# ChuyueL/advanced-hpc-lbm

Measured on NVIDIA B200. Metric: MLUPS (d2q9-bgk lattice updates per second / 1e6), higher is better.
Workload: dtype f32

## Files before the change

### advanced-hpc-lbm_b200/csrc/lbm_gpu.cu

```cuda
#include "lbm_gpu.h"
#include "lbm_kernels.cuh"
#include "lbm_cluster.cuh"
#include "lbm_tb2.cuh"
#include "lbm_tb3.cuh"
#include "lbm_pairs.cuh"
#include "lbm_f16.cuh"

#include <unistd.h>

#include <algorithm>
#include <cmath>
#include <cstdarg>
#include <cstdio>
#include <cstdlib>
#include <cstring>
#include <exception>
#include <memory>
#include <mutex>
#include <string>
#include <vector>

namespace {

thread_local std::string g_error;
// ... 1700 lines not shown
    s.rows = (int)nrows;
    const long long ar = (long long)params->ny - 2;
    s.accel_row = (ar >= row0 && ar < row0 + nrows) ? (int)(ar - row0) : LBM_NO_ROW;
    g->select_kernel();
    g->alloc_slab(s);
    if (g->kernel == LBM_GPU_KERNEL_TMA) g->make_tensor_maps(s);
    g->load_slab(s, cells_aos_rows, obstacles_rows, 0);
    if (nrows == params->ny) { g->connect_local(); g->prepare(); }
  } catch (const CudaError& e) {
    return fail("lbm_gpu_create_slab: %s", e.what.c_str());
  } catch (const std::exception& e) {
    return fail("lbm_gpu_create_slab: %s", e.what());
  }
  *out = reinterpret_cast<lbm_gpu*>(static_cast<GridBase*>(g.release()));
  return 0;
}

int lbm_gpu_ipc_export(lbm_gpu* h, void* desc) {
  if (!desc) return fail("lbm_gpu_ipc_export: NULL descriptor");
  return guarded<float>(h, "lbm_gpu_ipc_export", [&](Grid<float>& g) {
    if (g.slabs.size() != 1) throw CudaError{"only a one-slab handle can be exported"};
    if (g.f16) throw CudaError{"a LBM_GPU_STORE_F16 lattice cannot be shared between processes"};
    Slab<float>& s = g.slabs[0];
    CK(cudaSetDevice(s.device));
    IpcDesc d;
    memset(&d, 0, sizeof d);
    d.magic = kIpcMagic;
    d.elem_size = 4;
    d.device = s.device;
    d.pid = (int32_t)getpid();
    d.nx = g.prm.nx; d.pitch = g.pitch; d.rows = s.rows;
    d.row0 = s.row0;
    d.win_addr = (unsigned long long)(uintptr_t)s.win;
    d.win_bytes = s.win_bytes;
    d.off_sync = s.off_sync;
    d.off_gmask = s.off_gmask;
    d.steps_done = (unsigned long long)g.steps_done;
    d.passes_done = (unsigned long long)g.passes_done;
    d.local_free_cells = s.free_cells;
    d.cur = g.cur;
    d.tb2_ok = g.k7_fits(s.rows) ? 1 : 0;
    CK(cudaIpcGetMemHandle(&d.handle, s.win));
    cudaDeviceProp prop;
    CK(cudaGetDeviceProperties(&prop, s.device));
    memcpy(d.gpu_uuid, prop.uuid.bytes, 16);
    memset(desc, 0, LBM_GPU_IPC_DESC_BYTES);
    memcpy(desc, &d, sizeof d);
  });
}

namespace {
void ipc_connect_impl(Grid<float>& g, const IpcDesc& dn, const IpcDesc& up, bool ring_k7) {
  if (g.slabs.size() != 1) throw CudaError{"only a one-slab handle can be connected"};
  if (g.f16) throw CudaError{"a LBM_GPU_STORE_F16 lattice cannot be shared between processes"};
  Slab<float>& s = g.slabs[0];
  CK(cudaSetDevice(s.device));
  const long long ny = g.prm.ny;
  for (const IpcDesc* d : {&dn, &up}) {
    if (d->magic != kIpcMagic || d->elem_size != 4) throw CudaError{"bad neighbour descriptor"};
    if (d->nx != g.prm.nx || d->pitch != g.pitch) throw CudaError{"neighbour descriptor is for another grid width"};
    if (d->steps_done != (unsigned long long)g.steps_done || d->passes_done != (unsigned long long)g.passes_done ||
        d->cur != g.cur)
      throw CudaError{"neighbour is at a different timestep"};
  }
  cudaDeviceProp my_prop;
  CK(cudaGetDeviceProperties(&my_prop, s.device));
  for (const IpcDesc* d : {&dn, &up})
    if (memcmp(d->gpu_uuid, my_prop.uuid.bytes, 16) == 0 &&
        !(d->pid == (int32_t)getpid() && d->win_addr == (unsigned long long)(uintptr_t)s.win))
      throw CudaError{"a neighbouring slab runs on the same physical GPU: kernels that wait on one another "
                      "must not share a device (use lbm_gpu_create with n_gpus slabs in one process instead)"};
  if ((dn.row0 + dn.rows) % ny != s.row0 % ny) throw CudaError{"descriptor 'below' does not hold row0-1"};
  if ((s.row0 + s.rows) % ny != up.row0 % ny) throw CudaError{"descriptor 'above' does not hold row0+nrows"};
  auto map = [&](const IpcDesc& d, int slot) -> char* {
    if (d.pid == (int32_t)getpid()) {
      char* p = (char*)(uintptr_t)d.win_addr;
      if (p == s.win) return p;
      if (d.device == s.device)
        throw CudaError{"two slabs ordered by device-side flags must not share a GPU"};
      int can = 0;
      CK(cudaDeviceCanAccessPeer(&can, s.device, d.device));
      if (!can) throw CudaError{"peer access between the selected GPUs is not available"};
      cudaError_t e = cudaDeviceEnablePeerAccess(d.device, 0);
      if (e != cudaSuccess && e != cudaErrorPeerAccessAlreadyEnabled) CK(e);
      cudaGetLastError();
      return p;
    }
    if (g.use_pool()) {
      std::lock_guard<std::mutex> lock(g_window_mutex);
      for (auto& c : g_ipc_cache)
        if (c.device == s.device && memcmp(&c.handle, &d.handle, sizeof d.handle) == 0) return (char*)c.ptr;
    }
    void* p = nullptr;
    CK(cudaIpcOpenMemHandle(&p, d.handle, cudaIpcMemLazyEnablePeerAccess));
    if (g.use_pool()) {
      std::lock_guard<std::mutex> lock(g_window_mutex);
      g_ipc_cache.push_back({d.handle, s.device, p});
    } else {
      s.ipc_mapped[slot] = p;
    }
    return (char*)p;
  };
  for (const IpcDesc* d : {&dn, &up})
    if (d->win_bytes != s.win_bytes || d->off_sync != s.off_sync || d->off_gmask != s.off_gmask)
      throw CudaError{"neighbour window layout differs"};
  s.dn_win = map(dn, 0);
  s.up_win = (memcmp(&dn.handle, &up.handle, sizeof dn.handle) == 0 && dn.pid == up.pid) ? s.dn_win : map(up, 1);
  unsigned long long* dn_sync = (unsigned long long*)(s.dn_win + dn.off_sync);
  unsigned long long* up_sync = (unsigned long long*)(s.up_win + up.off_sync);
  s.dn_flag = dn_sync + kFlagFromAbove;
  s.up_flag = up_sync + kFlagFromBelow;
  s.dn_abort = dn_sync + kAbort;
  s.up_abort = up_sync + kAbort;
  s.dn_gmask = (uint32_t*)(s.dn_win + dn.off_gmask) + g.mask_pitch;
  s.up_gmask = (uint32_t*)(s.up_win + up.off_gmask);
  g.multi = true;
  g.use_flags = true;
  g.select_kernel(true, ring_k7);
  g.connected = true;
}
}

int lbm_gpu_ipc_connect(lbm_gpu* h, const void* desc_below, const void* desc_above) {
  if (!desc_below || !desc_above) return fail("lbm_gpu_ipc_connect: NULL descriptor");
  return guarded<float>(h, "lbm_gpu_ipc_connect", [&](Grid<float>& g) {
    IpcDesc dn, up;
    memcpy(&dn, desc_below, sizeof dn);
    memcpy(&up, desc_above, sizeof up);
    ipc_connect_impl(g, dn, up, false);
  });
}

int lbm_gpu_ipc_connect_all(lbm_gpu* h, const void* descs, int n) {
  if (!descs || n < 1) return fail("lbm_gpu_ipc_connect_all: bad argument");
  return guarded<float>(h, "lbm_gpu_ipc_connect_all", [&](Grid<float>& g) {
    if (g.slabs.size() != 1) throw CudaError{"only a one-slab handle can be connected"};
    Slab<float>& s = g.slabs[0];
    std::vector<IpcDesc> all(n);
    for (int i = 0; i < n; i++) memcpy(&all[i], (const char*)descs + (size_t)i * LBM_GPU_IPC_DESC_BYTES, sizeof(IpcDesc));
    const long long ny = g.prm.ny;
    long long rows_total = 0, free_total = 0;
    int below = -1, above = -1;
    bool all_k7 = true;
    for (int i = 0; i < n; i++) {
      const IpcDesc& d = all[i];
      if (d.magic != kIpcMagic) throw CudaError{"bad descriptor in the list"};
      rows_total += d.rows;
      free_total += d.local_free_cells;
      all_k7 = all_k7 && d.tb2_ok;
      if ((d.row0 + d.rows) % ny == s.row0 % ny) below = i;
      if ((s.row0 + s.rows) % ny == d.row0 % ny) above = i;
    }
    if (rows_total != ny) throw CudaError{"the descriptors do not cover the grid's rows exactly once"};
    if (below < 0 || above < 0) throw CudaError{"no descriptor holds the rows next to this slab"};
    ipc_connect_impl(g, all[below], all[above], all_k7);
    g.global_free_cells = free_total;
  });
}

int lbm_gpu_ipc_prepare(lbm_gpu* h) {
  return guarded<float>(h, "lbm_gpu_ipc_prepare", [&](Grid<float>& g) { g.prepare(); });
}

int lbm_gpu_run(lbm_gpu* h, int n_steps, float* av_vels_out) {
  return run_impl<float>(h, n_steps, av_vels_out, nullptr, "lbm_gpu_run");
}
int lbm_gpu_run_f64(lbm_gpu* h, int n_steps, double* av_vels_out) {
  return run_impl<double>(h, n_steps, av_vels_out, nullptr, "lbm_gpu_run_f64");
}
int lbm_gpu_run_batch(lbm_gpu* const* handles, int n, int n_steps, float* av_vels_out) {
  return run_batch_impl(handles, n, n_steps, av_vels_out);
}
int lbm_gpu_run_sums(lbm_gpu* h, int n_steps, double* sums_out) {
  if (!h) return fail("lbm_gpu_run_sums: NULL handle");
  if (reinterpret_cast<GridBase*>(h)->is_f64()) return run_impl<double>(h, n_steps, nullptr, sums_out, "lbm_gpu_run_sums");
  return run_impl<float>(h, n_steps, nullptr, sums_out, "lbm_gpu_run_sums");
}

int lbm_gpu_set_global_free_cells(lbm_gpu* h, long long free_cells) {
  if (!h) return fail("lbm_gpu_set_global_free_cells: NULL handle");
  if (free_cells < 1) return fail("lbm_gpu_set_global_free_cells: count must be positive");
  GridBase* b = reinterpret_cast<GridBase*>(h);
  if (b->is_f64()) static_cast<Grid<double>*>(b)->global_free_cells = free_cells;
  else static_cast<Grid<float>*>(b)->global_free_cells = free_cells;
  return 0;
}

int lbm_gpu_download(lbm_gpu* h, float* out) {
  if (!out) return fail("lbm_gpu_download: NULL output");
  return guarded<float>(h, "lbm_gpu_download", [&](Grid<float>& g) {
    long long rows = 0;
    for (auto& s : g.slabs) rows += s.rows;
    g.download_rows(g.slabs[0].row0, rows, out);
  });
}
int lbm_gpu_download_f64(lbm_gpu* h, double* out) {
  if (!out) return fail("lbm_gpu_download_f64: NULL output");
  return guarded<double>(h, "lbm_gpu_download_f64", [&](Grid<double>& g) {
    long long rows = 0;
    for (auto& s : g.slabs) rows += s.rows;
    g.download_rows(g.slabs[0].row0, rows, out);
  });
}
int lbm_gpu_download_rows(lbm_gpu* h, long long row0, long long nrows, float* out) {
  if (!out || nrows < 0) return fail("lbm_gpu_download_rows: bad argument");
  return guarded<float>(h, "lbm_gpu_download_rows", [&](Grid<float>& g) { g.download_rows(row0, nrows, out); });
}

int lbm_gpu_final_fields(lbm_gpu* h, long long row0, long long nrows, float* ux, float* uy, float* u, float* p) {
  if (nrows < 0) return fail("lbm_gpu_final_fields: bad argument");
  return guarded<float>(h, "lbm_gpu_final_fields", [&](Grid<float>& g) { g.final_fields(row0, nrows, ux, uy, u, p); });
}
int lbm_gpu_final_fields_f64(lbm_gpu* h, long long row0, long long nrows, double* ux, double* uy, double* u, double* p) {
  if (nrows < 0) return fail("lbm_gpu_final_fields_f64: bad argument");
  return guarded<double>(h, "lbm_gpu_final_fields_f64", [&](Grid<double>& g) { g.final_fields(row0, nrows, ux, uy, u, p); });
}

int lbm_gpu_av_velocity(lbm_gpu* h, float* av_out) {
  if (!av_out) return fail("lbm_gpu_av_velocity: NULL output");
  return guarded<float>(h, "lbm_gpu_av_velocity", [&](Grid<float>& g) {
    *av_out = (float)(g.av_velocity_sum() / (double)g.divisor());
  });
}
int lbm_gpu_av_velocity_f64(lbm_gpu* h, double* av_out) {
  if (!av_out) return fail("lbm_gpu_av_velocity_f64: NULL output");
  return guarded<double>(h, "lbm_gpu_av_velocity_f64", [&](Grid<double>& g) {
    *av_out = g.av_velocity_sum() / (double)g.divisor();
  });
}

int lbm_gpu_digest(lbm_gpu* h, double* total_density, unsigned long long* checksum) {
  if (!h) return fail("lbm_gpu_digest: NULL handle");
  if (reinterpret_cast<GridBase*>(h)->is_f64())
    return guarded<double>(h, "lbm_gpu_digest", [&](Grid<double>& g) { g.digest(total_density, checksum); });
  return guarded<float>(h, "lbm_gpu_digest", [&](Grid<float>& g) { g.digest(total_density, checksum); });
}

int lbm_gpu_upload(lbm_gpu* h, const float* cells_aos) {
  if (!cells_aos) return fail("lbm_gpu_upload: NULL input");
  return guarded<float>(h, "lbm_gpu_upload", [&](Grid<float>& g) {
    const int cur = g.cur;
    const long long base = g.slabs[0].row0;
    for (auto& s : g.slabs) g.upload_cells(s, cells_aos + (size_t)(s.row0 - base) * g.prm.nx * 9, cur);
    if (!g.slab_mode || g.slabs[0].rows == g.prm.ny) g.prepare();
  });
}
int lbm_gpu_upload_f64(lbm_gpu* h, const double* cells_aos) {
  if (!cells_aos) return fail("lbm_gpu_upload_f64: NULL input");
  return guarded<double>(h, "lbm_gpu_upload_f64", [&](Grid<double>& g) {
    const int cur = g.cur;
    for (auto& s : g.slabs) g.upload_cells(s, cells_aos + (size_t)s.row0 * g.prm.nx * 9, cur);
    g.prepare();
  });
}

int lbm_gpu_get_info(lbm_gpu* h, lbm_gpu_info* info) {
  if (!h || !info) return fail("lbm_gpu_get_info: NULL argument");
  memset(info, 0, sizeof *info);
  GridBase* b = reinterpret_cast<GridBase*>(h);
  auto fill = [&](auto& g) {
    info->nx = g.prm.nx; info->ny = g.prm.ny;
    info->n_gpus = (int)g.slabs.size();
    info->is_f64 = g.is_f64();
    info->kernel = g.kernel;
    info->pitch = g.pitch;
    info->local_free_cells = g.local_free_cells();
    info->free_cells = g.divisor();
    info->local_row0 = g.slabs[0].row0;
    long long rows = 0;
    size_t bytes = 0;
    for (auto& s : g.slabs) { rows += s.rows; bytes = std::max(bytes, s.bytes + kStagingBytes); }
    info->local_rows = rows;
    info->steps_done = g.steps_done;
    info->kernel_launches = g.launches;
    info->last_run_device_ms = g.last_run_ms;
    info->last_step_kernel_ms = g.last_step_ms;
    info->device_bytes = bytes;
  };
  if (b->is_f64()) fill(*static_cast<Grid<double>*>(b));
  else fill(*static_cast<Grid<float>*>(b));
  return 0;
}

int lbm_gpu_host_alloc(size_t bytes, void** out) {
  if (!out) return fail("lbm_gpu_host_alloc: NULL argument");
  *out = nullptr;
  cudaError_t e = cudaHostAlloc(out, bytes, cudaHostAllocPortable);
  if (e != cudaSuccess) {
    cudaGetLastError();
    return fail("lbm_gpu_host_alloc: %s", cudaGetErrorString(e));
  }
  return 0;
}

void lbm_gpu_host_free(void* p) {
  if (p) cudaFreeHost(p);
}

void lbm_gpu_destroy(lbm_gpu* h) {
  if (!h) return;
  delete reinterpret_cast<GridBase*>(h);
}

}
```

### advanced-hpc-lbm_b200/csrc/lbm_tb2.cuh

```cuda
#pragma once
#include "lbm_kernels.cuh"

namespace lbm {

#ifndef LBM_TB2_THREADS
#define LBM_TB2_THREADS 96
#endif
#define LBM_TB2_SPAN (LBM_TB2_THREADS * 4)
#define LBM_TB2_PAD 4
#define LBM_TB2_ROWF (LBM_TB2_SPAN + 2 * LBM_TB2_PAD)
#define LBM_TB2_MAX_WOUT (LBM_TB2_SPAN - 8)
#ifndef LBM_TB2_MIN_BLOCKS
#define LBM_TB2_MIN_BLOCKS 4
#endif

struct Tb2Smem {
  float in[2][9][LBM_TB2_ROWF];
  float r013[2][3][LBM_TB2_ROWF];
  float r256[3][3][LBM_TB2_ROWF];
  float r78[2][LBM_TB2_ROWF];
  unsigned long long mbar[2];
  unsigned long long mbar_free;
};
static_assert(sizeof(Tb2Smem) * LBM_TB2_MIN_BLOCKS <= 225 * 1024, "LBM_TB2_MIN_BLOCKS blocks of shared memory per SM");
static_assert((LBM_TB2_ROWF * sizeof(float)) % 16 == 0, "staged rows must keep 16-byte alignment");

struct Tb2Args {
  StepArgs<float> s;
  const uint32_t* ghost_mask;
  unsigned long long* av2;
  int wout;
  int span;
  int seg_rows;
  int n_big;
  int big_rows;
  int seg_rows_tail;
  unsigned long long* av3;
};

__device__ __forceinline__ void tb2_mbar_wait(unsigned long long* bar, const uint32_t parity) {
  const uint32_t addr = smem_u32(bar);
  uint32_t done = 0;
  while (!done)
    asm volatile("{ .reg .pred p; mbarrier.try_wait.parity.shared::cta.b64 p, [%1], %2; selp.b32 %0, 1, 0, p; }"
                 : "=r"(done) : "r"(addr), "r"(parity) : "memory");
}

__device__ __forceinline__ void tb2_bulk_load(float* dst_smem, const float* src, const uint32_t bytes,
                                              unsigned long long* bar) {
  asm volatile("cp.async.bulk.shared::cluster.global.mbarrier::complete_tx::bytes [%0], [%1], %2, [%3];"
               ::"r"(smem_u32(dst_smem)), "l"(src), "r"(bytes), "r"(smem_u32(bar)) : "memory");
}

template <bool PERIODIC = false>
__device__ __forceinline__ const float* tb2_row_ptr(const StepArgs<float>& a, const int k, int row) {
  if (PERIODIC) {
    row = (row < 0) ? row + a.rows : (row >= a.rows) ? row - a.rows : row;
  } else {
    if (row < 0) return a.ghost_s + (long long)((-1 - row) * 9 + k) * a.pitch;
    if (row >= a.rows) return a.ghost_n + (long long)((row - a.rows) * 9 + k) * a.pitch;
  }
  if (row == a.accel_row && k != 0 && k != 2 && k != 4) {
    const int idx = (k == 1) ? 0 : (k == 3) ? 1 : k - 3;
    return a.side_src + (long long)idx * a.pitch;
  }
  return a.src + (long long)k * a.plane_stride + (long long)row * a.pitch;
}

template <typename Smem>
__device__ __forceinline__ void tb2_expect(Smem& sm, const int stage, const int span) {
  asm volatile("mbarrier.arrive.expect_tx.shared::cta.b64 _, [%0], %1;" ::"r"(smem_u32(&sm.mbar[stage])),
               "r"((uint32_t)(9 * span * sizeof(float))) : "memory");
}
__device__ __forceinline__ int tb2_plane_of_thread() {
  const int nwarps = (int)blockDim.x >> 5, w = (int)threadIdx.x >> 5, lane = (int)threadIdx.x & 31;
  const int k = w + nwarps * lane;
  return (k < 9) ? k : -1;
}
template <bool PERIODIC = false, typename Smem>
__device__ __forceinline__ void tb2_issue(const StepArgs<float>& a, Smem& sm, const int stage, const int r,
                                          const int s0, const int span, const int k) {
  if (k < 0) return;
  unsigned long long* bar = &sm.mbar[stage];
  const int dy = (k == 2 || k == 5 || k == 6) ? -1 : (k == 4 || k == 7 || k == 8) ? 1 : 0;
  const float* row = tb2_row_ptr<PERIODIC>(a, k, r + dy);
  float* dst = &sm.in[stage][k][LBM_TB2_PAD];
  int col = s0, left = span;
  while (left > 0) {
    const int n = min(left, a.nx - col);
    tb2_bulk_load(dst, row + col, (uint32_t)n * 4u, bar);
    dst += n;
    left -= n;
    col = 0;
  }
}

__device__ __forceinline__ void tb2_get(const float* row, const int c0, float& v0, float& v1, float& v2, float& v3) {
  const float4 v = *reinterpret_cast<const float4*>(row + LBM_TB2_PAD + c0);
  v0 = v.x; v1 = v.y; v2 = v.z; v3 = v.w;
}
__device__ __forceinline__ void tb2_get_west(const float* row, const int c0, float& v0, float& v1, float& v2, float& v3) {
  const float4 v = *reinterpret_cast<const float4*>(row + LBM_TB2_PAD + c0);
  v0 = row[LBM_TB2_PAD + c0 - 1]; v1 = v.x; v2 = v.y; v3 = v.z;
}
__device__ __forceinline__ void tb2_get_east(const float* row, const int c0, float& v0, float& v1, float& v2, float& v3) {
  const float4 v = *reinterpret_cast<const float4*>(row + LBM_TB2_PAD + c0);
  v0 = v.y; v1 = v.z; v2 = v.w; v3 = row[LBM_TB2_PAD + c0 + 4];
}
__device__ __forceinline__ void tb2_ring_read_done(Tb2Smem& sm) {
  __syncwarp();
  if ((threadIdx.x & 31) == 0)
    asm volatile("mbarrier.arrive.shared::cta.b64 _, [%0];" ::"r"(smem_u32(&sm.mbar_free)) : "memory");
}
__device__ __forceinline__ void tb2_put(float* row, const int c0, const float (&o)[4][9], const int k) {
  *reinterpret_cast<float4*>(row + LBM_TB2_PAD + c0) = make_float4(o[0][k], o[1][k], o[2][k], o[3][k]);
}

template <bool STRICT>
__device__ __forceinline__ void tb2_store_row(const StepArgs<float>& a, const int y, const int xg, float (&out)[4][9],
                                              const uint32_t mbits) {
  const long long PS = a.plane_stride;
  float* d = a.dst + (long long)y * a.pitch + xg;
#pragma unroll
  for (int k = 0; k < 9; k++)
    *reinterpret_cast<float4*>(d + k * PS) = make_float4(out[0][k], out[1][k], out[2][k], out[3][k]);
  const bool first = (y == 0), second = (y == 1), last = (y == a.rows - 1), before_last = (y == a.rows - 2);
  const bool cA = (y == a.accel_row);
  if (first | second | last | before_last | cA) {
    if (cA) {
#pragma unroll
      for (int j = 0; j < 4; j++)
        cell_accelerate<float, STRICT>(out[j][1], out[j][3], out[j][5], out[j][6], out[j][7], out[j][8],
                                       (mbits >> j) & 1u, a.aw1, a.aw2);
      const int ks[6] = {1, 3, 5, 6, 7, 8};
#pragma unroll
      for (int n = 0; n < 6; n++)
        *reinterpret_cast<float4*>(a.side_dst + (long long)n * a.pitch + xg) =
            make_float4(out[0][ks[n]], out[1][ks[n]], out[2][ks[n]], out[3][ks[n]]);
    }
#define LBM_TB2_PUSH(dst, depth, k)                                                             \
  *reinterpret_cast<float4*>((dst) + (long long)((depth) * 9 + (k)) * a.pitch + xg) =          \
      make_float4(out[0][k], out[1][k], out[2][k], out[3][k]);
    if (first) {
      LBM_TB2_PUSH(a.push_dn, 0, 4) LBM_TB2_PUSH(a.push_dn, 0, 7) LBM_TB2_PUSH(a.push_dn, 0, 8)
      LBM_TB2_PUSH(a.push_dn, 0, 0) LBM_TB2_PUSH(a.push_dn, 0, 1) LBM_TB2_PUSH(a.push_dn, 0, 3)
    }
    if (last) {
      LBM_TB2_PUSH(a.push_up, 0, 2) LBM_TB2_PUSH(a.push_up, 0, 5) LBM_TB2_PUSH(a.push_up, 0, 6)
      LBM_TB2_PUSH(a.push_up, 0, 0) LBM_TB2_PUSH(a.push_up, 0, 1) LBM_TB2_PUSH(a.push_up, 0, 3)
    }
    if (second) { LBM_TB2_PUSH(a.push_dn, 1, 4) LBM_TB2_PUSH(a.push_dn, 1, 7) LBM_TB2_PUSH(a.push_dn, 1, 8) }
    if (before_last) { LBM_TB2_PUSH(a.push_up, 1, 2) LBM_TB2_PUSH(a.push_up, 1, 5) LBM_TB2_PUSH(a.push_up, 1, 6) }
#undef LBM_TB2_PUSH
  }
}

template <bool STRICT>
__device__ __forceinline__ void tb2_tile(const Tb2Args& ta, Tb2Smem& sm, const int strip, const int seg,
                                         uint32_t& phases, unsigned long long& q1, unsigned long long& q2,
                                         bool& bad1, bool& bad2) {
  const StepArgs<float>& a = ta.s;
  const int tid = threadIdx.x;
  const int X0 = strip * ta.wout;
  const int S0 = (X0 >= LBM_TB2_PAD) ? X0 - LBM_TB2_PAD : X0 - LBM_TB2_PAD + a.nx;
  const bool big = seg < ta.n_big;
  const int R0 = big ? seg * ta.seg_rows : ta.big_rows + (seg - ta.n_big) * ta.seg_rows_tail;
  const int R1 = big ? min(R0 + ta.seg_rows, ta.big_rows) : min(R0 + ta.seg_rows_tail, a.rows);
  const int n_it = R1 - R0 + 2;

  const int c0 = min(4 * tid, ta.span - 4);
  int xg = S0 + c0;
  while (xg >= a.nx) xg -= a.nx;
  const bool owned = (tid >= 1) && (4 * tid < ta.span) && (c0 - LBM_TB2_PAD < ta.wout) &&
                     (X0 + c0 - LBM_TB2_PAD < a.nx);

  const int my_plane = tb2_plane_of_thread();
  if (tid == 0) { tb2_expect(sm, 0, ta.span); tb2_expect(sm, 1, ta.span); }
#pragma unroll 1
  for (int k = 0; k < 2; k++) tb2_issue(a, sm, k, R0 - 1 + k, S0, ta.span, my_plane);

  const QuadConsts<float, STRICT> qc(a.omega);
  const int mword_idx = xg >> 5, mshift = xg & 31;
  auto mask_bits = [&](const int row) -> uint32_t {
    const uint32_t* m = (row < 0) ? ta.ghost_mask : (row >= a.rows) ? ta.ghost_mask + a.mask_pitch
                                                                    : a.mask + (long long)row * a.mask_pitch;
    return (m[mword_idx] >> mshift) & 0xFu;
  };
  uint32_t mbits = mask_bits(R0 - 1);
  uint32_t mbits_prev = 0u;

#pragma unroll 1
  for (int i = 0; i < n_it; i++) {
    const int st = i & 1;
    const int r = R0 - 1 + i;
    const uint32_t mbits_next = (i + 1 < n_it) ? mask_bits(r + 1) : 0u;
    float keep4[4];
    {
      tb2_mbar_wait(&sm.mbar[st], (phases >> st) & 1u);
      phases ^= 1u << st;
      if (tid == 0 && i + 2 < n_it) tb2_expect(sm, st, ta.span);
      float in[4][9], out[4][9];
      const float(*row)[LBM_TB2_ROWF] = sm.in[st];
      tb2_get(row[0], c0, in[0][0], in[1][0], in[2][0], in[3][0]);
      tb2_get(row[2], c0, in[0][2], in[1][2], in[2][2], in[3][2]);
      tb2_get(row[4], c0, in[0][4], in[1][4], in[2][4], in[3][4]);
      tb2_get_west(row[1], c0, in[0][1], in[1][1], in[2][1], in[3][1]);
      tb2_get_west(row[5], c0, in[0][5], in[1][5], in[2][5], in[3][5]);
      tb2_get_west(row[8], c0, in[0][8], in[1][8], in[2][8], in[3][8]);
      tb2_get_east(row[3], c0, in[0][3], in[1][3], in[2][3], in[3][3]);
      tb2_get_east(row[6], c0, in[0][6], in[1][6], in[2][6], in[3][6]);
      tb2_get_east(row[7], c0, in[0][7], in[1][7], in[2][7], in[3][7]);
      bool bad;
      const unsigned long long q = quad_update<float, STRICT>(in, mbits, qc, out, bad);
      if (owned && r >= R0 && r < R1) { q1 += q; bad1 |= bad; }
      if (r == a.accel_row) {
#pragma unroll
        for (int j = 0; j < 4; j++)
          cell_accelerate<float, STRICT>(out[j][1], out[j][3], out[j][5], out[j][6], out[j][7], out[j][8],
                                         (mbits >> j) & 1u, a.aw1, a.aw2);
      }
      if (i > 0) {
        tb2_mbar_wait(&sm.mbar_free, (phases >> 2) & 1u);
        phases ^= 4u;
      }
      tb2_put(sm.r013[i & 1][0], c0, out, 0);
      tb2_put(sm.r013[i & 1][1], c0, out, 1);
      tb2_put(sm.r013[i & 1][2], c0, out, 3);
      tb2_put(sm.r256[i % 3][0], c0, out, 2);
      tb2_put(sm.r256[i % 3][1], c0, out, 5);
      tb2_put(sm.r256[i % 3][2], c0, out, 6);
      tb2_put(sm.r78[0], c0, out, 7);
      tb2_put(sm.r78[1], c0, out, 8);
#pragma unroll
      for (int j = 0; j < 4; j++) keep4[j] = out[j][4];
    }
    __syncthreads();
    if (i + 2 < n_it) tb2_issue(a, sm, st, r + 2, S0, ta.span, my_plane);

    if (i >= 2) {
      const int y = r - 1;
      float in[4][9], out[4][9];
      const float(*c)[LBM_TB2_ROWF] = sm.r013[(i - 1) & 1];
      const float(*s)[LBM_TB2_ROWF] = sm.r256[(i - 2) % 3];
      tb2_get(c[0], c0, in[0][0], in[1][0], in[2][0], in[3][0]);
      tb2_get_west(c[1], c0, in[0][1], in[1][1], in[2][1], in[3][1]);
      tb2_get_east(c[2], c0, in[0][3], in[1][3], in[2][3], in[3][3]);
      tb2_get(s[0], c0, in[0][2], in[1][2], in[2][2], in[3][2]);
      tb2_get_west(s[1], c0, in[0][5], in[1][5], in[2][5], in[3][5]);
      tb2_get_east(s[2], c0, in[0][6], in[1][6], in[2][6], in[3][6]);
#pragma unroll
      for (int j = 0; j < 4; j++) in[j][4] = keep4[j];
      tb2_get_east(sm.r78[0], c0, in[0][7], in[1][7], in[2][7], in[3][7]);
      tb2_get_west(sm.r78[1], c0, in[0][8], in[1][8], in[2][8], in[3][8]);
      tb2_ring_read_done(sm);
      bool bad;
      const unsigned long long q = quad_update<float, STRICT>(in, mbits_prev, qc, out, bad);
      if (owned) {
        q2 += q;
        bad2 |= bad;
        tb2_store_row<STRICT>(a, y, xg, out, mbits_prev);
      }
    }
    else {
      tb2_ring_read_done(sm);
    }
    mbits_prev = mbits;
    mbits = mbits_next;
  }

}

__device__ __forceinline__ void tb2_init_smem(Tb2Smem& sm, const int span) {
  const int tid = threadIdx.x;
  for (int i = tid; i < 35 * 2 * LBM_TB2_PAD; i += blockDim.x) {
    float* row = &sm.in[0][0][0] + (size_t)(i / (2 * LBM_TB2_PAD)) * LBM_TB2_ROWF;
    const int e = i % (2 * LBM_TB2_PAD);
    row[e < LBM_TB2_PAD ? e : span + e] = 0.f;
  }
  if (tid == 0) {
    asm volatile("mbarrier.init.shared::cta.b64 [%0], 1;" ::"r"(smem_u32(&sm.mbar[0])) : "memory");
    asm volatile("mbarrier.init.shared::cta.b64 [%0], 1;" ::"r"(smem_u32(&sm.mbar[1])) : "memory");
    asm volatile("mbarrier.init.shared::cta.b64 [%0], %1;" ::"r"(smem_u32(&sm.mbar_free)), "r"((uint32_t)(blockDim.x >> 5)) : "memory");
    asm volatile("fence.mbarrier_init.release.cluster;" ::: "memory");
  }
}

template <bool STRICT, bool MULTI>
__global__ void __launch_bounds__(LBM_TB2_THREADS, LBM_TB2_MIN_BLOCKS)
lbm_step2_tb(const __grid_constant__ Tb2Args ta) {
  extern __shared__ __align__(128) unsigned char tb2_smem_raw[];
  Tb2Smem& sm = *reinterpret_cast<Tb2Smem*>(tb2_smem_raw);
  const StepArgs<float>& a = ta.s;
  int strip, seg;
  tile_of_block(a.tiles_x, a.tiles_y, 1, strip, seg);
  const bool is_boundary = is_edge_tile(seg, a.tiles_y, 1);
  tb2_init_smem(sm, ta.span);
  cudaGridDependencySynchronize();
  __syncthreads();
  boundary_wait<float, MULTI>(a, is_boundary);
  uint32_t phases = 0u;
  unsigned long long q1 = 0ULL, q2 = 0ULL;
  bool bad1 = false, bad2 = false;
  tb2_tile<STRICT>(ta, sm, strip, seg, phases, q1, q2, bad1, bad2);
  if (bad1) atomicOr(a.av + 1, LBM_NONFINITE_MARK);
  if (bad2) atomicOr(ta.av2 + 1, LBM_NONFINITE_MARK);
  block_accumulate(q1, a.av);
  __syncthreads();
  block_accumulate(q2, ta.av2);
  boundary_signal<float, MULTI>(a, is_boundary);
}

}
```

### advanced-hpc-lbm_b200/csrc/lbm_tb3.cuh

```cuda
#pragma once
#include "lbm_tb2.cuh"

namespace lbm {

#ifndef LBM_TB3_MIN_BLOCKS
#define LBM_TB3_MIN_BLOCKS (LBM_TB2_THREADS <= 64 ? 4 : LBM_TB2_THREADS <= 96 ? 3 : 2)
#endif

struct Tb3Level {
  float r13[2][2][LBM_TB2_ROWF];
  float r56[3][2][LBM_TB2_ROWF];
  float r78[2][LBM_TB2_ROWF];
};
struct Tb3Smem {
  float in[2][9][LBM_TB2_ROWF];
  Tb3Level lv[2];
  float p0[2][LBM_TB2_ROWF];
  unsigned long long mbar[2];
};
constexpr int kTb3PlaneRows = 18 + 2 * 12 + 2;
static_assert(sizeof(Tb3Smem) == kTb3PlaneRows * LBM_TB2_ROWF * sizeof(float) + 16, "ring layout");
static_assert((sizeof(Tb3Smem) + 512 + 1024) * LBM_TB3_MIN_BLOCKS <= 228 * 1024,
              "LBM_TB3_MIN_BLOCKS blocks of shared memory per SM");

__device__ __forceinline__ void tb3_init_smem(Tb3Smem& sm, const int span) {
  const int tid = threadIdx.x;
  for (int i = tid; i < kTb3PlaneRows * 2 * LBM_TB2_PAD; i += blockDim.x) {
    float* row = &sm.in[0][0][0] + (size_t)(i / (2 * LBM_TB2_PAD)) * LBM_TB2_ROWF;
    const int e = i % (2 * LBM_TB2_PAD);
    row[e < LBM_TB2_PAD ? e : span + e] = 0.f;
  }
  if (tid == 0) {
    asm volatile("mbarrier.init.shared::cta.b64 [%0], 1;" ::"r"(smem_u32(&sm.mbar[0])) : "memory");
    asm volatile("mbarrier.init.shared::cta.b64 [%0], 1;" ::"r"(smem_u32(&sm.mbar[1])) : "memory");
    asm volatile("fence.mbarrier_init.release.cluster;" ::: "memory");
  }
}

__device__ __forceinline__ void tb3_gather(const Tb3Level& L, const int c0, const int s13, const int s56,
                                           const float (&p0)[4], const float (&p2)[4], const float (&p4)[4],
                                           float (&in)[4][9]) {
#pragma unroll
  for (int j = 0; j < 4; j++) { in[j][0] = p0[j]; in[j][2] = p2[j]; in[j][4] = p4[j]; }
  tb2_get_west(L.r13[s13][0], c0, in[0][1], in[1][1], in[2][1], in[3][1]);
  tb2_get_east(L.r13[s13][1], c0, in[0][3], in[1][3], in[2][3], in[3][3]);
  tb2_get_west(L.r56[s56][0], c0, in[0][5], in[1][5], in[2][5], in[3][5]);
  tb2_get_east(L.r56[s56][1], c0, in[0][6], in[1][6], in[2][6], in[3][6]);
  tb2_get_east(L.r78[0], c0, in[0][7], in[1][7], in[2][7], in[3][7]);
  tb2_get_west(L.r78[1], c0, in[0][8], in[1][8], in[2][8], in[3][8]);
}
__device__ __forceinline__ void tb3_put_level(Tb3Level& L, const int c0, const int i, const float (&o)[4][9]) {
  tb2_put(L.r13[i & 1][0], c0, o, 1);
  tb2_put(L.r13[i & 1][1], c0, o, 3);
  tb2_put(L.r56[i % 3][0], c0, o, 5);
  tb2_put(L.r56[i % 3][1], c0, o, 6);
  tb2_put(L.r78[0], c0, o, 7);
  tb2_put(L.r78[1], c0, o, 8);
}

template <bool STRICT>
__device__ __forceinline__ void tb3_accelerate(const StepArgs<float>& a, float (&o)[4][9], const uint32_t mbits) {
#pragma unroll
  for (int j = 0; j < 4; j++)
    cell_accelerate<float, STRICT>(o[j][1], o[j][3], o[j][5], o[j][6], o[j][7], o[j][8], (mbits >> j) & 1u, a.aw1, a.aw2);
}

struct Tb3Carry {
  float p0[4];
  float p2a[4];
  float p2b[4];
  __device__ __forceinline__ void shift(const float (&o)[4][9]) {
#pragma unroll
    for (int j = 0; j < 4; j++) { p0[j] = o[j][0]; p2a[j] = p2b[j]; p2b[j] = o[j][2]; }
  }
};

template <bool STRICT>
__device__ __forceinline__ void tb3_tile(const Tb2Args& ta, Tb3Smem& sm, const int strip, const int seg,
                                         unsigned long long (&q)[3], bool (&bad)[3]) {
  const StepArgs<float>& a = ta.s;
  const int tid = threadIdx.x;
  const int X0 = strip * ta.wout;
  const int S0 = (X0 >= LBM_TB2_PAD) ? X0 - LBM_TB2_PAD : X0 - LBM_TB2_PAD + a.nx;
  const bool big = seg < ta.n_big;
  const int R0 = big ? seg * ta.seg_rows : ta.big_rows + (seg - ta.n_big) * ta.seg_rows_tail;
  const int R1 = big ? min(R0 + ta.seg_rows, ta.big_rows) : min(R0 + ta.seg_rows_tail, a.rows);
  const int n_it = R1 - R0 + 4;

  const int c0 = min(4 * tid, ta.span - 4);
  int xg = S0 + c0;
  while (xg >= a.nx) xg -= a.nx;
  const bool owned = (tid >= 1) && (4 * tid < ta.span) && (c0 - LBM_TB2_PAD < ta.wout) &&
                     (X0 + c0 - LBM_TB2_PAD < a.nx);

  const int my_plane = tb2_plane_of_thread();
  if (tid == 0) { tb2_expect(sm, 0, ta.span); tb2_expect(sm, 1, ta.span); }
#pragma unroll 1
  for (int k = 0; k < 2; k++) tb2_issue<true>(a, sm, k, R0 - 2 + k, S0, ta.span, my_plane);

  const QuadConsts<float, STRICT> qc(a.omega);
  const int mword_idx = xg >> 5, mshift = xg & 31;
  auto wrap = [&](const int row) { return (row < 0) ? row + a.rows : (row >= a.rows) ? row - a.rows : row; };
  auto mask_bits = [&](const int row) -> uint32_t {
    return (a.mask[(long long)wrap(row) * a.mask_pitch + mword_idx] >> mshift) & 0xFu;
  };
  uint32_t m1 = mask_bits(R0 - 2), m2 = 0u, m3 = 0u;
  Tb3Carry c1, c2;
  uint32_t phases = 0u;

#pragma unroll 1
  for (int i = 0; i < n_it; i++) {
    const int st = i & 1;
    const int r = R0 - 2 + i;
    const uint32_t m_next = (i + 1 < n_it) ? mask_bits(r + 1) : 0u;
    float in[4][9], out[4][9];
    bool b;
    tb2_mbar_wait(&sm.mbar[st], (phases >> st) & 1u);
    phases ^= 1u << st;
    if (tid == 0 && i + 2 < n_it) tb2_expect(sm, st, ta.span);
    {
      const float(*row)[LBM_TB2_ROWF] = sm.in[st];
      tb2_get(row[0], c0, in[0][0], in[1][0], in[2][0], in[3][0]);
      tb2_get(row[2], c0, in[0][2], in[1][2], in[2][2], in[3][2]);
      tb2_get(row[4], c0, in[0][4], in[1][4], in[2][4], in[3][4]);
      tb2_get_west(row[1], c0, in[0][1], in[1][1], in[2][1], in[3][1]);
      tb2_get_west(row[5], c0, in[0][5], in[1][5], in[2][5], in[3][5]);
      tb2_get_west(row[8], c0, in[0][8], in[1][8], in[2][8], in[3][8]);
      tb2_get_east(row[3], c0, in[0][3], in[1][3], in[2][3], in[3][3]);
      tb2_get_east(row[6], c0, in[0][6], in[1][6], in[2][6], in[3][6]);
      tb2_get_east(row[7], c0, in[0][7], in[1][7], in[2][7], in[3][7]);
    }
    unsigned long long qq = quad_update<float, STRICT>(in, m1, qc, out, b);
    if (owned && r >= R0 && r < R1) { q[0] += qq; bad[0] |= b; }
    if (wrap(r) == a.accel_row) tb3_accelerate<STRICT>(a, out, m1);
    tb3_put_level(sm.lv[0], c0, i, out);
    float p4[4];
#pragma unroll
    for (int j = 0; j < 4; j++) p4[j] = out[j][4];
    __syncthreads();
    if (i + 2 < n_it) tb2_issue<true>(a, sm, st, r + 2, S0, ta.span, my_plane);

    if (i >= 2) {
      const int y = r - 1;
      tb3_gather(sm.lv[0], c0, (i - 1) & 1, (i - 2) % 3, c1.p0, c1.p2a, p4, in);
      c1.shift(out);
      qq = quad_update<float, STRICT>(in, m2, qc, out, b);
      if (owned && y >= R0 && y < R1) { q[1] += qq; bad[1] |= b; }
      if (wrap(y) == a.accel_row) tb3_accelerate<STRICT>(a, out, m2);
      tb3_put_level(sm.lv[1], c0, i, out);
      tb2_put(sm.p0[i & 1], c0, out, 0);
      float n2[4];
#pragma unroll
      for (int j = 0; j < 4; j++) { n2[j] = out[j][2]; p4[j] = out[j][4]; }
      __syncthreads();

      if (i >= 4) {
        const int z = r - 2;
        tb3_gather(sm.lv[1], c0, (i - 1) & 1, (i - 2) % 3, c2.p2a, c2.p2a, p4, in);
        tb2_get(sm.p0[(i - 1) & 1], c0, in[0][0], in[1][0], in[2][0], in[3][0]);
        qq = quad_update<float, STRICT>(in, m3, qc, out, b);
        if (owned) {
          q[2] += qq;
          bad[2] |= b;
          tb2_store_row<STRICT>(a, z, xg, out, m3);
        }
      }
#pragma unroll
      for (int j = 0; j < 4; j++) { c2.p2a[j] = c2.p2b[j]; c2.p2b[j] = n2[j]; }
    } else {
      c1.shift(out);
    }
    m3 = m2;
    m2 = m1;
    m1 = m_next;
  }
}

template <bool STRICT>
__global__ void __launch_bounds__(LBM_TB2_THREADS, LBM_TB3_MIN_BLOCKS)
lbm_step3_tb(const __grid_constant__ Tb2Args ta) {
  extern __shared__ __align__(128) unsigned char tb3_smem_raw[];
  Tb3Smem& sm = *reinterpret_cast<Tb3Smem*>(tb3_smem_raw);
  const StepArgs<float>& a = ta.s;
  int strip, seg;
  tile_of_block(a.tiles_x, a.tiles_y, 1, strip, seg);
  tb3_init_smem(sm, ta.span);
  cudaGridDependencySynchronize();
  __syncthreads();
  unsigned long long q[3] = {0ULL, 0ULL, 0ULL};
  bool bad[3] = {false, false, false};
  tb3_tile<STRICT>(ta, sm, strip, seg, q, bad);
  if (bad[0]) atomicOr(a.av + 1, LBM_NONFINITE_MARK);
  if (bad[1]) atomicOr(ta.av2 + 1, LBM_NONFINITE_MARK);
  if (bad[2]) atomicOr(ta.av3 + 1, LBM_NONFINITE_MARK);
  block_accumulate(q[0], a.av);
  __syncthreads();
  block_accumulate(q[1], ta.av2);
  __syncthreads();
  block_accumulate(q[2], ta.av3);
}

}
```

Measured before the change: 176,000.

## Unroll tb3 row loop by stage phase with compile-time ring slots and incremental indexing

Restructures the three-level temporal-blocking loop into compile-time-specialized iterations (prologue stages plus a 2-way unrolled steady state), so buffer slots and stage guards become constants. It replaces per-row modulo/wrap arithmetic for mask and accel rows with incremental pointers and a rotating ring offset, and splits edge/halo stores out so the common row store is a plain streaming write. It also drops the tail-segment path, assuming uniform segments, and adds compile-gated timing/no-compute experiment hooks that are off by default. The intent is to cut integer overhead and branching in the inner loop at the cost of larger code.

```diff
diff --git a/advanced-hpc-lbm_b200/csrc/lbm_gpu.cu b/advanced-hpc-lbm_b200/csrc/lbm_gpu.cu
--- a/advanced-hpc-lbm_b200/csrc/lbm_gpu.cu
+++ b/advanced-hpc-lbm_b200/csrc/lbm_gpu.cu
@@ -2026,4 +2026,14 @@
   delete reinterpret_cast<GridBase*>(h);
 }
 
-}
+#if LBM_TB3_EXPERIMENT == 2
+int lbm_gpu_experiment_tb3_cycles(unsigned long long* out) {
+  const unsigned long long zero[5] = {0, 0, 0, 0, 0};
+  if (cudaMemcpyFromSymbol(out, lbm::tb3_cycles, sizeof(zero)) != cudaSuccess ||
+      cudaMemcpyToSymbol(lbm::tb3_cycles, zero, sizeof(zero)) != cudaSuccess)
+    return fail("lbm_gpu_experiment_tb3_cycles: %s", cudaGetErrorString(cudaGetLastError()));
+  return 0;
+}
+#endif
+
+}
diff --git a/advanced-hpc-lbm_b200/csrc/lbm_tb2.cuh b/advanced-hpc-lbm_b200/csrc/lbm_tb2.cuh
--- a/advanced-hpc-lbm_b200/csrc/lbm_tb2.cuh
+++ b/advanced-hpc-lbm_b200/csrc/lbm_tb2.cuh
@@ -117,13 +117,8 @@
 }
 
 template <bool STRICT>
-__device__ __forceinline__ void tb2_store_row(const StepArgs<float>& a, const int y, const int xg, float (&out)[4][9],
-                                              const uint32_t mbits) {
-  const long long PS = a.plane_stride;
-  float* d = a.dst + (long long)y * a.pitch + xg;
-#pragma unroll
-  for (int k = 0; k < 9; k++)
-    *reinterpret_cast<float4*>(d + k * PS) = make_float4(out[0][k], out[1][k], out[2][k], out[3][k]);
+__device__ __forceinline__ void tb2_store_edges(const StepArgs<float>& a, const int y, const int xg, float (&out)[4][9],
+                                                const uint32_t mbits) {
   const bool first = (y == 0), second = (y == 1), last = (y == a.rows - 1), before_last = (y == a.rows - 2);
   const bool cA = (y == a.accel_row);
   if (first | second | last | before_last | cA) {
@@ -153,6 +148,16 @@
     if (before_last) { LBM_TB2_PUSH(a.push_up, 1, 2) LBM_TB2_PUSH(a.push_up, 1, 5) LBM_TB2_PUSH(a.push_up, 1, 6) }
 #undef LBM_TB2_PUSH
   }
+}
+template <bool STRICT>
+__device__ __forceinline__ void tb2_store_row(const StepArgs<float>& a, const int y, const int xg, float (&out)[4][9],
+                                              const uint32_t mbits) {
+  const long long PS = a.plane_stride;
+  float* d = a.dst + (long long)y * a.pitch + xg;
+#pragma unroll
+  for (int k = 0; k < 9; k++)
+    *reinterpret_cast<float4*>(d + k * PS) = make_float4(out[0][k], out[1][k], out[2][k], out[3][k]);
+  tb2_store_edges<STRICT>(a, y, xg, out, mbits);
 }
 
 template <bool STRICT>
diff --git a/advanced-hpc-lbm_b200/csrc/lbm_tb3.cuh b/advanced-hpc-lbm_b200/csrc/lbm_tb3.cuh
--- a/advanced-hpc-lbm_b200/csrc/lbm_tb3.cuh
+++ b/advanced-hpc-lbm_b200/csrc/lbm_tb3.cuh
@@ -1,10 +1,27 @@
 #pragma once
+#include <type_traits>
 #include "lbm_tb2.cuh"
 
 namespace lbm {
 
 #ifndef LBM_TB3_MIN_BLOCKS
 #define LBM_TB3_MIN_BLOCKS (LBM_TB2_THREADS <= 64 ? 4 : LBM_TB2_THREADS <= 96 ? 3 : 2)
+#endif
+#ifdef LBM_EXPERIMENTS
+#ifndef LBM_TB3_EXPERIMENT
+#define LBM_TB3_EXPERIMENT 0
+#endif
+#else
+#ifdef LBM_TB3_EXPERIMENT
+#error "LBM_TB3_EXPERIMENT needs -DLBM_EXPERIMENTS"
+#endif
+#define LBM_TB3_EXPERIMENT 0
+#endif
+#if LBM_TB3_EXPERIMENT == 2
+__device__ unsigned long long tb3_cycles[5];
+#define LBM_TB3_TIMED(acc, ...) do { const uint32_t t0_ = (uint32_t)clock(); __VA_ARGS__; acc += (uint32_t)clock() - t0_; } while (0)
+#else
+#define LBM_TB3_TIMED(acc, ...) do { __VA_ARGS__; } while (0)
 #endif
 
 struct Tb3Level {
@@ -37,23 +54,24 @@
   }
 }
 
-__device__ __forceinline__ void tb3_gather(const Tb3Level& L, const int c0, const int s13, const int s56,
+__device__ __forceinline__ void tb3_gather(const Tb3Level& L, const int c0, const int s13, const int o56,
                                            const float (&p0)[4], const float (&p2)[4], const float (&p4)[4],
                                            float (&in)[4][9]) {
 #pragma unroll
   for (int j = 0; j < 4; j++) { in[j][0] = p0[j]; in[j][2] = p2[j]; in[j][4] = p4[j]; }
   tb2_get_west(L.r13[s13][0], c0, in[0][1], in[1][1], in[2][1], in[3][1]);
   tb2_get_east(L.r13[s13][1], c0, in[0][3], in[1][3], in[2][3], in[3][3]);
-  tb2_get_west(L.r56[s56][0], c0, in[0][5], in[1][5], in[2][5], in[3][5]);
-  tb2_get_east(L.r56[s56][1], c0, in[0][6], in[1][6], in[2][6], in[3][6]);
+  tb2_get_west(L.r56[0][0] + o56, c0, in[0][5], in[1][5], in[2][5], in[3][5]);
+  tb2_get_east(L.r56[0][1] + o56, c0, in[0][6], in[1][6], in[2][6], in[3][6]);
   tb2_get_east(L.r78[0], c0, in[0][7], in[1][7], in[2][7], in[3][7]);
   tb2_get_west(L.r78[1], c0, in[0][8], in[1][8], in[2][8], in[3][8]);
 }
-__device__ __forceinline__ void tb3_put_level(Tb3Level& L, const int c0, const int i, const float (&o)[4][9]) {
-  tb2_put(L.r13[i & 1][0], c0, o, 1);
-  tb2_put(L.r13[i & 1][1], c0, o, 3);
-  tb2_put(L.r56[i % 3][0], c0, o, 5);
-  tb2_put(L.r56[i % 3][1], c0, o, 6);
+__device__ __forceinline__ void tb3_put_level(Tb3Level& L, const int c0, const int s13, const int o56,
+                                              const float (&o)[4][9]) {
+  tb2_put(L.r13[s13][0], c0, o, 1);
+  tb2_put(L.r13[s13][1], c0, o, 3);
+  tb2_put(L.r56[0][0] + o56, c0, o, 5);
+  tb2_put(L.r56[0][1] + o56, c0, o, 6);
   tb2_put(L.r78[0], c0, o, 7);
   tb2_put(L.r78[1], c0, o, 8);
 }
@@ -63,6 +81,22 @@
 #pragma unroll
   for (int j = 0; j < 4; j++)
     cell_accelerate<float, STRICT>(o[j][1], o[j][3], o[j][5], o[j][6], o[j][7], o[j][8], (mbits >> j) & 1u, a.aw1, a.aw2);
+}
+
+template <bool STRICT>
+__device__ __forceinline__ unsigned long long tb3_update(const float (&in)[4][9], const uint32_t mbits,
+                                                         const QuadConsts<float, STRICT>& qc, float (&out)[4][9],
+                                                         bool& bad) {
+#if LBM_TB3_EXPERIMENT == 1
+#pragma unroll
+  for (int j = 0; j < 4; j++)
+#pragma unroll
+    for (int k = 0; k < 9; k++) out[j][k] = in[j][k];
+  bad = false;
+  return mbits;
+#else
+  return quad_update<float, STRICT>(in, mbits, qc, out, bad);
+#endif
 }
 
 struct Tb3Carry {
@@ -74,6 +108,8 @@
     for (int j = 0; j < 4; j++) { p0[j] = o[j][0]; p2a[j] = p2b[j]; p2b[j] = o[j][2]; }
   }
 };
+
+template <int V> using Tb3Int = std::integral_constant<int, V>;
 
 template <bool STRICT>
 __device__ __forceinline__ void tb3_tile(const Tb2Args& ta, Tb3Smem& sm, const int strip, const int seg,
@@ -82,44 +118,58 @@
   const int tid = threadIdx.x;
   const int X0 = strip * ta.wout;
   const int S0 = (X0 >= LBM_TB2_PAD) ? X0 - LBM_TB2_PAD : X0 - LBM_TB2_PAD + a.nx;
-  const bool big = seg < ta.n_big;
-  const int R0 = big ? seg * ta.seg_rows : ta.big_rows + (seg - ta.n_big) * ta.seg_rows_tail;
-  const int R1 = big ? min(R0 + ta.seg_rows, ta.big_rows) : min(R0 + ta.seg_rows_tail, a.rows);
+  const int R0 = seg * ta.seg_rows;
+  const int R1 = min(R0 + ta.seg_rows, ta.big_rows);
   const int n_it = R1 - R0 + 4;
-
-  const int c0 = min(4 * tid, ta.span - 4);
+  const int rows = a.rows, span = ta.span;
+
+  const int c0 = min(4 * tid, span - 4);
   int xg = S0 + c0;
   while (xg >= a.nx) xg -= a.nx;
-  const bool owned = (tid >= 1) && (4 * tid < ta.span) && (c0 - LBM_TB2_PAD < ta.wout) &&
+  const bool owned = (tid >= 1) && (4 * tid < span) && (c0 - LBM_TB2_PAD < ta.wout) &&
                      (X0 + c0 - LBM_TB2_PAD < a.nx);
 
   const int my_plane = tb2_plane_of_thread();
-  if (tid == 0) { tb2_expect(sm, 0, ta.span); tb2_expect(sm, 1, ta.span); }
+  if (tid == 0) { tb2_expect(sm, 0, span); tb2_expect(sm, 1, span); }
 #pragma unroll 1
-  for (int k = 0; k < 2; k++) tb2_issue<true>(a, sm, k, R0 - 2 + k, S0, ta.span, my_plane);
+  for (int k = 0; k < 2; k++) tb2_issue<true>(a, sm, k, R0 - 2 + k, S0, span, my_plane);
 
   const QuadConsts<float, STRICT> qc(a.omega);
-  const int mword_idx = xg >> 5, mshift = xg & 31;
-  auto wrap = [&](const int row) { return (row < 0) ? row + a.rows : (row >= a.rows) ? row - a.rows : row; };
-  auto mask_bits = [&](const int row) -> uint32_t {
-    return (a.mask[(long long)wrap(row) * a.mask_pitch + mword_idx] >> mshift) & 0xFu;
+  const int mshift = xg & 31;
+  const int msize = rows * a.mask_pitch;
+  int rw = (R0 >= 2) ? R0 - 2 : R0 - 2 + rows;
+  int mo = rw * a.mask_pitch + (xg >> 5);
+  auto next_mask = [&]() -> uint32_t {
+    const uint32_t m = (__ldg(a.mask + mo) >> mshift) & 0xFu;
+    mo += a.mask_pitch;
+    if (mo >= msize) mo -= msize;
+    return m;
   };
-  uint32_t m1 = mask_bits(R0 - 2), m2 = 0u, m3 = 0u;
+  uint32_t m1 = next_mask(), m2 = 0u, m3 = 0u;
+  uint32_t acc = 0u;
+  float* drow = a.dst + (long long)R0 * a.pitch + xg;
+  const long long PS = a.plane_stride;
   Tb3Carry c1, c2;
   uint32_t phases = 0u;
-
-#pragma unroll 1
-  for (int i = 0; i < n_it; i++) {
-    const int st = i & 1;
-    const int r = R0 - 2 + i;
-    const uint32_t m_next = (i + 1 < n_it) ? mask_bits(r + 1) : 0u;
+  int s56 = 0, s56_old = 2 * LBM_TB2_ROWF, s56_mid = 4 * LBM_TB2_ROWF;
+#if LBM_TB3_EXPERIMENT == 2
+  uint32_t cyc[3] = {0u, 0u, 0u};
+  const uint32_t t_tile = (uint32_t)clock();
+#endif
+
+  auto iteration = [&](const int i, auto st_c, auto sub_c) {
+    constexpr int ST = decltype(st_c)::value, SUB = decltype(sub_c)::value;
+    const uint32_t m_next = next_mask();
+    acc = (acc << 1) | (rw == a.accel_row ? 1u : 0u);
+    rw = (rw + 1 == rows) ? 0 : rw + 1;
     float in[4][9], out[4][9];
     bool b;
-    tb2_mbar_wait(&sm.mbar[st], (phases >> st) & 1u);
-    phases ^= 1u << st;
-    if (tid == 0 && i + 2 < n_it) tb2_expect(sm, st, ta.span);
+    LBM_TB3_TIMED(cyc[0], tb2_mbar_wait(&sm.mbar[ST], (phases >> ST) & 1u));
+    phases ^= 1u << ST;
+    const bool refill = i + 2 < n_it;
+    if (tid == 0 && refill) tb2_expect(sm, ST, span);
     {
-      const float(*row)[LBM_TB2_ROWF] = sm.in[st];
+      const float(*row)[LBM_TB2_ROWF] = sm.in[ST];
       tb2_get(row[0], c0, in[0][0], in[1][0], in[2][0], in[3][0]);
       tb2_get(row[2], c0, in[0][2], in[1][2], in[2][2], in[3][2]);
       tb2_get(row[4], c0, in[0][4], in[1][4], in[2][4], in[3][4]);
@@ -130,50 +180,77 @@
       tb2_get_east(row[6], c0, in[0][6], in[1][6], in[2][6], in[3][6]);
       tb2_get_east(row[7], c0, in[0][7], in[1][7], in[2][7], in[3][7]);
     }
-    unsigned long long qq = quad_update<float, STRICT>(in, m1, qc, out, b);
-    if (owned && r >= R0 && r < R1) { q[0] += qq; bad[0] |= b; }
-    if (wrap(r) == a.accel_row) tb3_accelerate<STRICT>(a, out, m1);
-    tb3_put_level(sm.lv[0], c0, i, out);
+    unsigned long long qq = tb3_update<STRICT>(in, m1, qc, out, b);
+    if (SUB > 1 && owned && i < n_it - 2) { q[0] += qq; bad[0] |= b; }
+    if (acc & 1u) tb3_accelerate<STRICT>(a, out, m1);
+    tb3_put_level(sm.lv[0], c0, ST, s56, out);
     float p4[4];
 #pragma unroll
     for (int j = 0; j < 4; j++) p4[j] = out[j][4];
-    __syncthreads();
-    if (i + 2 < n_it) tb2_issue<true>(a, sm, st, r + 2, S0, ta.span, my_plane);
-
-    if (i >= 2) {
-      const int y = r - 1;
-      tb3_gather(sm.lv[0], c0, (i - 1) & 1, (i - 2) % 3, c1.p0, c1.p2a, p4, in);
+    LBM_TB3_TIMED(cyc[1], __syncthreads());
+    if (refill) tb2_issue<true>(a, sm, ST, R0 + i, S0, span, my_plane);
+
+    if constexpr (SUB == 1) {
       c1.shift(out);
-      qq = quad_update<float, STRICT>(in, m2, qc, out, b);
-      if (owned && y >= R0 && y < R1) { q[1] += qq; bad[1] |= b; }
-      if (wrap(y) == a.accel_row) tb3_accelerate<STRICT>(a, out, m2);
-      tb3_put_level(sm.lv[1], c0, i, out);
-      tb2_put(sm.p0[i & 1], c0, out, 0);
+    } else {
+      tb3_gather(sm.lv[0], c0, ST ^ 1, s56_old, c1.p0, c1.p2a, p4, in);
+      c1.shift(out);
+      qq = tb3_update<STRICT>(in, m2, qc, out, b);
+      if (owned && i >= 3 && i < n_it - 1) { q[1] += qq; bad[1] |= b; }
+      if (acc & 2u) tb3_accelerate<STRICT>(a, out, m2);
+      tb3_put_level(sm.lv[1], c0, ST, s56, out);
+      tb2_put(sm.p0[ST], c0, out, 0);
       float n2[4];
 #pragma unroll
       for (int j = 0; j < 4; j++) { n2[j] = out[j][2]; p4[j] = out[j][4]; }
-      __syncthreads();
-
-      if (i >= 4) {
-        const int z = r - 2;
-        tb3_gather(sm.lv[1], c0, (i - 1) & 1, (i - 2) % 3, c2.p2a, c2.p2a, p4, in);
-        tb2_get(sm.p0[(i - 1) & 1], c0, in[0][0], in[1][0], in[2][0], in[3][0]);
-        qq = quad_update<float, STRICT>(in, m3, qc, out, b);
+      LBM_TB3_TIMED(cyc[2], __syncthreads());
+
+      if constexpr (SUB == 3) {
+        tb3_gather(sm.lv[1], c0, ST ^ 1, s56_old, c2.p2a, c2.p2a, p4, in);
+        tb2_get(sm.p0[ST ^ 1], c0, in[0][0], in[1][0], in[2][0], in[3][0]);
+        qq = tb3_update<STRICT>(in, m3, qc, out, b);
         if (owned) {
           q[2] += qq;
           bad[2] |= b;
-          tb2_store_row<STRICT>(a, z, xg, out, m3);
+#pragma unroll
+          for (int k = 0; k < 9; k++)
+            *reinterpret_cast<float4*>(drow + k * PS) = make_float4(out[0][k], out[1][k], out[2][k], out[3][k]);
+          const int z = R0 - 4 + i;
+          if ((acc & 4u) || (unsigned)(z - 2) >= (unsigned)(rows - 4))
+            tb2_store_edges<STRICT>(a, z, xg, out, m3);
         }
+        drow += a.pitch;
       }
 #pragma unroll
       for (int j = 0; j < 4; j++) { c2.p2a[j] = c2.p2b[j]; c2.p2b[j] = n2[j]; }
-    } else {
-      c1.shift(out);
     }
     m3 = m2;
     m2 = m1;
     m1 = m_next;
-  }
+    const int s = s56;
+    s56 = s56_old;
+    s56_old = s56_mid;
+    s56_mid = s;
+  };
+
+  iteration(0, Tb3Int<0>(), Tb3Int<1>());
+  iteration(1, Tb3Int<1>(), Tb3Int<1>());
+  iteration(2, Tb3Int<0>(), Tb3Int<2>());
+  iteration(3, Tb3Int<1>(), Tb3Int<2>());
+  int i = 4;
+#pragma unroll 1
+  for (; i + 1 < n_it; i += 2) {
+    iteration(i, Tb3Int<0>(), Tb3Int<3>());
+    iteration(i + 1, Tb3Int<1>(), Tb3Int<3>());
+  }
+  if (i < n_it) iteration(i, Tb3Int<0>(), Tb3Int<3>());
+#if LBM_TB3_EXPERIMENT == 2
+  if (blockIdx.x % 16 == 0 && (tid & 31) == 0) {
+    for (int k = 0; k < 3; k++) atomicAdd(&tb3_cycles[k], (unsigned long long)cyc[k]);
+    atomicAdd(&tb3_cycles[3], (unsigned long long)((uint32_t)clock() - t_tile));
+    atomicAdd(&tb3_cycles[4], 1ULL);
+  }
+#endif
 }
 
 template <bool STRICT>
```

Result: faster. 209,400, median of 6 (+18.9%).
